# agent-charon/MinGraph-UNet

Measured on AMD Instinct MI355X. Metric: segmented Mpix/sec, full MinGraph-UNet forward (U-Net + patch-graph GAT), 512x512 batch, higher is better.
Workload: dtype f32

## Files before the change

### mingraph-unet_amd/csrc/convt_x3.hip

```cpp
#include <hip/hip_runtime.h>
#include <stdint.h>

#include <algorithm>
#include <type_traits>

#include "common.h"
#include "pack_small.h"

namespace mgu {

typedef float f32x16 __attribute__((ext_vector_type(16)));
typedef float f32x4 __attribute__((ext_vector_type(4)));
typedef unsigned u32x4 __attribute__((ext_vector_type(4)));
typedef __bf16 bf16x8 __attribute__((ext_vector_type(8)));

namespace {

__device__ __forceinline__ void split3_pack(const float a, const float b, unsigned& p0, unsigned& p1, unsigned& p2) {
  const unsigned ua = __float_as_uint(a), ub = __float_as_uint(b);
  p0 = __builtin_amdgcn_perm(ub, ua, 0x07060302u);
  const float ra = a - __uint_as_float(ua & 0xffff0000u), rb = b - __uint_as_float(ub & 0xffff0000u);
  const unsigned va = __float_as_uint(ra), vb = __float_as_uint(rb);
  p1 = __builtin_amdgcn_perm(vb, va, 0x07060302u);
  const float sa = ra - __uint_as_float(va & 0xffff0000u), sb = rb - __uint_as_float(vb & 0xffff0000u);
  p2 = __builtin_amdgcn_perm(__float_as_uint(sb), __float_as_uint(sa), 0x07060302u);
}

__device__ __forceinline__ f32x16 mfma_bf16(const u32x4 a, const u32x4 b, const f32x16 c) {
  return __builtin_amdgcn_mfma_f32_32x32x16_bf16(__builtin_bit_cast(bf16x8, a), __builtin_bit_cast(bf16x8, b), c, 0, 0, 0);
}

__global__ void pack_convt_x3_kernel(const float* __restrict__ w, uint16_t* __restrict__ Wx, int Cin, int Cout) {
  pack_convt_x3_body(w, Wx, Cin, Cout, 0, blockIdx.x, gridDim.x);
}

__device__ __forceinline__ void lds_barrier() { asm volatile("s_waitcnt lgkmcnt(0)\n\ts_barrier" ::: "memory"); }

template <int MODE, int NI>
__global__ __launch_bounds__(256, 2) void convt2x2_x3_kernel(const float* __restrict__ in, const int ldin, const uint16_t* __restrict__ Wx,
                                                             const float* __restrict__ shift, float* __restrict__ out, const int M,
                                                             const int H, const int W, const int Cin, const int Cout, const int ldout,
                                                             const int coff, const int Hout, const int Wout, const int ntn,
                                                             const int nblocks) {
  constexpr int AP = 40, ABUF = 3 * 128 * AP;
  __shared__ __attribute__((aligned(16))) uint16_t As[2 * ABUF];
  __shared__ int rowoff[128];
  const int chunk = gridDim.x >> 3;
  const int lb = (blockIdx.x & 7) * chunk + (blockIdx.x >> 3);
  if (lb >= nblocks) return;
  const int nt = lb % ntn, mt = lb / ntn;
  const int tid = threadIdx.x, lane = tid & 63, wave = tid >> 6;
  const int wm = wave >> 1, wn = wave & 1, lr = lane & 31, lh = lane >> 5;
  const int bm0 = mt * 128;
  const int HW = H * W;
  long long pix0;
  {
    const int img = bm0 / HW, rem = bm0 - img * HW, y = rem / W;
    pix0 = ((long long)img * Hout + 2 * y) * Wout + 2 * (rem - y * W);
  }
  if (tid < 128) {
    const int m = bm0 + tid;
    int off = 0;
    if (m < M) {
      const int img = m / HW, rem = m - img * HW, y = rem / W, x = rem - y * W;
      off = (int)((((long long)img * Hout + 2 * y) * Wout + 2 * x - pix0) * ldout);
    }
    rowoff[tid] = off;
  }

  const int arow = tid >> 3, ach = (tid & 7) * 4;
  const float* aptr[4];
#pragma unroll
  for (int j = 0; j < 4; ++j) {
    const int m = min(bm0 + j * 32 + arow, M - 1);
    if (MODE == 0) {
      aptr[j] = in + (size_t)m * ldin + ach;
    } else {
      const int img = m / HW, rem = m - img * HW, y = rem / W, x = rem - y * W;
      aptr[j] = in + (((size_t)img * Hout + 2 * y) * Wout + 2 * x) * ldin + ach;
    }
  }
  const int nk = (MODE == 0 ? Cin : 4 * Cin) >> 5;
  const int spq = Cin >> 5;
  auto koff = [&](int s) -> int {
    if (MODE == 0) return s * 32;
    const int q = s / spq;
    return ((q >> 1) * Wout + (q & 1)) * ldin + (s - q * spq) * 32;
  };
  f32x4 areg[2][4];
  auto load_a = [&](int s, auto set_t) {
    constexpr int set = decltype(set_t)::value;
    const int ko = koff(s);
#pragma unroll
    for (int j = 0; j < 4; ++j) areg[set][j] = *reinterpret_cast<const f32x4*>(aptr[j] + ko);
  };
  auto store_a = [&](int buf, auto set_t) {
    constexpr int set = decltype(set_t)::value;
    uint16_t* const base = As + buf * ABUF + arow * AP + ach;
#pragma unroll
    for (int j = 0; j < 4; ++j) {
      unsigned p[3][2];
      split3_pack(areg[set][j][0], areg[set][j][1], p[0][0], p[1][0], p[2][0]);
      split3_pack(areg[set][j][2], areg[set][j][3], p[0][1], p[1][1], p[2][1]);
#pragma unroll
      for (int q = 0; q < 3; ++q) *reinterpret_cast<uint2*>(base + (q * 128 + j * 32) * AP) = uint2{p[q][0], p[q][1]};
    }
  };

  const int nt128 = NI == 2 ? nt : nt >> 1, sub0 = NI == 2 ? wn * 2 : (nt & 1) * 2 + wn;
  const u32x4* const bp = reinterpret_cast<const u32x4*>(Wx) + ((size_t)nt128 * (2 * nk) * 12 + sub0 * 3) * 64 + lane;
  u32x4 br[2][3 * NI];
  auto load_b = [&](int kk, auto buf_t) {
    constexpr int buf = decltype(buf_t)::value;
#pragma unroll
    for (int f = 0; f < 3 * NI; ++f) br[buf][f] = bp[((size_t)kk * 12 + f) * 64];
  };

  f32x16 acc[2][NI];
#pragma unroll
  for (int mi = 0; mi < 2; ++mi)
#pragma unroll
    for (int ni = 0; ni < NI; ++ni)
#pragma unroll
      for (int r = 0; r < 16; ++r) acc[mi][ni][r] = 0.f;

  const int aoff = (wm * 64 + lr) * AP + lh * 8;
  auto half_step = [&](int buf, int ss, auto bb_t) {
    constexpr int bb = decltype(bb_t)::value;
    u32x4 pa[2][3];
#pragma unroll
    for (int mi = 0; mi < 2; ++mi)
#pragma unroll
      for (int q = 0; q < 3; ++q)
        pa[mi][q] = *reinterpret_cast<const u32x4*>(As + buf * ABUF + (q * 128 + mi * 32) * AP + aoff + ss * 16);
#pragma unroll
    for (int mi = 0; mi < 2; ++mi)
#pragma unroll
      for (int ni = 0; ni < NI; ++ni) {
        f32x16 t = acc[mi][ni];
        t = mfma_bf16(pa[mi][2], br[bb][ni * 3 + 0], t);
        t = mfma_bf16(pa[mi][0], br[bb][ni * 3 + 2], t);
        t = mfma_bf16(pa[mi][1], br[bb][ni * 3 + 1], t);
        t = mfma_bf16(pa[mi][1], br[bb][ni * 3 + 0], t);
        t = mfma_bf16(pa[mi][0], br[bb][ni * 3 + 1], t);
        t = mfma_bf16(pa[mi][0], br[bb][ni * 3 + 0], t);
        acc[mi][ni] = t;
      }
  };
  using B0 = std::integral_constant<int, 0>;
  using B1 = std::integral_constant<int, 1>;
  const int nkk = 2 * nk;
  load_a(0, B0{});
  load_a(min(1, nk - 1), B1{});
  load_b(0, B0{});
  store_a(0, B0{});
  lds_barrier();
  auto second_half_and_stage = [&](int buf, auto bb_t, auto set_t) {
    half_step(buf, 1, bb_t);
    store_a(buf ^ 1, set_t);
#pragma unroll
    for (int k = 0; k < 12 * NI; ++k) {
      __builtin_amdgcn_sched_group_barrier(0x008, 1, 0);
      __builtin_amdgcn_sched_group_barrier(0x002, NI == 2 ? 4 : 8, 0);
    }
    __builtin_amdgcn_sched_group_barrier(0x200, 12, 0);
  };
  for (int s = 0; s < nk; s += 2) {
    load_a(min(s + 2, nk - 1), B0{});
    load_b(min(2 * s + 1, nkk - 1), B1{});
    __builtin_amdgcn_sched_barrier(0);
    half_step(0, 0, B0{});
    load_b(min(2 * s + 2, nkk - 1), B0{});
    __builtin_amdgcn_sched_barrier(0);
    second_half_and_stage(0, B1{}, B1{});
    __builtin_amdgcn_sched_barrier(0);
    lds_barrier();
    if (s + 1 >= nk) break;
    load_a(min(s + 3, nk - 1), B1{});
    load_b(min(2 * s + 3, nkk - 1), B1{});
    __builtin_amdgcn_sched_barrier(0);
    half_step(1, 0, B0{});
    load_b(min(2 * s + 4, nkk - 1), B0{});
    __builtin_amdgcn_sched_barrier(0);
    second_half_and_stage(1, B1{}, B0{});
    __builtin_amdgcn_sched_barrier(0);
    lds_barrier();
  }

  float* const tile_out = MODE == 0 ? out + (size_t)pix0 * ldout + coff : out + (size_t)bm0 * ldout + coff;
  const bool full_m = bm0 + 128 <= M;
  auto store_tile = [&](auto guarded_t) {
    constexpr bool GUARDED = decltype(guarded_t)::value;
#pragma unroll
    for (int ni = 0; ni < NI; ++ni) {
      const int n = nt * (64 * NI) + wn * (32 * NI) + ni * 32 + lr;
      int ncol = n;
      if (MODE == 0) {
        const int q = n / Cout;
        ncol = ((q >> 1) * Wout + (q & 1)) * ldout + (n - q * Cout);
      }
      const float sh = shift ? shift[n] : 0.f;
#pragma unroll
      for (int mi = 0; mi < 2; ++mi)
#pragma unroll
        for (int r = 0; r < 16; ++r) {
          const int rrow = wm * 64 + mi * 32 + (r & 3) + 8 * (r >> 2) + 4 * lh;
          const unsigned idx = (unsigned)((MODE == 0 ? rowoff[rrow] : rrow * ldout) + ncol);
          const float v = acc[mi][ni][r] + sh;
          if (!GUARDED) tile_out[idx] = v;
          else if (bm0 + rrow < M) tile_out[idx] = v;
        }
    }
  };
  if (full_m) store_tile(std::false_type{});
  else store_tile(std::true_type{});
}

}

size_t convt_x3_floats(int Cin, int Cout) { return (size_t)Cin * Cout * 6; }


namespace {

__global__ void pack_convt_x3_dgrad_kernel(const float* __restrict__ w, uint16_t* __restrict__ Wx, int Cin, int Cout) {
  pack_convt_x3_body(w, Wx, Cin, Cout, 1, blockIdx.x, gridDim.x);
}

}

size_t convt_x3_dgrad_floats(int Cin, int Cout) { return (size_t)((Cin + 127) / 128 * 128) * Cout * 6; }

hipError_t launch_pack_convt_x3_dgrad(const float* w, float* Wx, int Cin, int Cout, hipStream_t s) {
  if ((Cin & 63) || (Cout & 31)) return hipErrorInvalidValue;
  hipLaunchKernelGGL(pack_convt_x3_dgrad_kernel, dim3((unsigned)std::min<int64_t>(4096, ((int64_t)Cin * Cout * 4 + 255) / 256)), dim3(256), 0, s, w,
                     reinterpret_cast<uint16_t*>(Wx), Cin, Cout);
  return hipGetLastError();
}

hipError_t launch_convt_x3_dgrad(const IgemmDesc& d, hipStream_t s) {
  const bool wide = (d.N & 127) == 0;
  const int mtiles = (d.M + 127) / 128, ntn = d.N / (wide ? 128 : 64);
  const int nb = mtiles * ntn;
  const int chunk = (nb + 7) / 8;
  if (wide)
    hipLaunchKernelGGL((convt2x2_x3_kernel<1, 2>), dim3(chunk * 8), dim3(256), 0, s, d.in, d.ldin, reinterpret_cast<const uint16_t*>(d.wu),
                       (const float*)nullptr, d.out, d.M, d.H, d.W, d.Cp, d.N, d.ldout, d.coff, d.Hout, d.Wout, ntn, nb);
  else
    hipLaunchKernelGGL((convt2x2_x3_kernel<1, 1>), dim3(chunk * 8), dim3(256), 0, s, d.in, d.ldin, reinterpret_cast<const uint16_t*>(d.wu),
                       (const float*)nullptr, d.out, d.M, d.H, d.W, d.Cp, d.N, d.ldout, d.coff, d.Hout, d.Wout, ntn, nb);
  return hipGetLastError();
}

hipError_t launch_pack_convt_x3(const float* w, float* Wx, int Cin, int Cout, hipStream_t s) {
  if ((Cin & 15) || (Cout & 31)) return hipErrorInvalidValue;
  hipLaunchKernelGGL(pack_convt_x3_kernel, dim3((unsigned)std::min<int64_t>(4096, ((int64_t)Cin * Cout * 4 + 255) / 256)), dim3(256), 0, s, w, reinterpret_cast<uint16_t*>(Wx), Cin,
                     Cout);
  return hipGetLastError();
}

hipError_t launch_convt_x3(const IgemmDesc& d, hipStream_t s) {
  const int mtiles = (d.M + 127) / 128, ntn = d.N / 128;
  const int nb = mtiles * ntn;
  const int chunk = (nb + 7) / 8;
  hipLaunchKernelGGL((convt2x2_x3_kernel<0, 2>), dim3(chunk * 8), dim3(256), 0, s, d.in, d.ldin, reinterpret_cast<const uint16_t*>(d.wu), d.shift, d.out,
                     d.M, d.H, d.W, d.Cp, d.ct_cout, d.ldout, d.coff, d.Hout, d.Wout, ntn, nb);
  return hipGetLastError();
}

}
```

Before: 798.0.

## Make transposed-conv x3 kernel persistent with cross-tile prefetch and LDS-staged stores

Specializes the MODE 0, NI 2 transposed-conv kernel into a persistent kernel. Grid size is capped at the resident workgroup count and each workgroup loops over its XCD chunk of tiles, prefetching the next tile's A and B operands while the current tile's epilogue runs. The epilogue transposes accumulators through LDS so that stores are 4-wide contiguous per row instead of scattered scalar writes. This targets launch-tail and epilogue overhead and store coalescing, at the cost of extra LDS traffic, more scheduling complexity and a host-side occupancy query cached per device.

```diff
diff --git a/mingraph-unet_amd/csrc/convt_x3.hip b/mingraph-unet_amd/csrc/convt_x3.hip
--- a/mingraph-unet_amd/csrc/convt_x3.hip
+++ b/mingraph-unet_amd/csrc/convt_x3.hip
@@ -2,6 +2,7 @@
 #include <stdint.h>
 
 #include <algorithm>
+#include <atomic>
 #include <type_traits>
 
 #include "common.h"
@@ -35,6 +36,12 @@
 }
 
 __device__ __forceinline__ void lds_barrier() { asm volatile("s_waitcnt lgkmcnt(0)\n\ts_barrier" ::: "memory"); }
+__device__ __forceinline__ void lds_barrier_fenced() {
+  asm volatile("" ::: "memory");
+  __builtin_amdgcn_s_waitcnt(0xC07F);
+  __builtin_amdgcn_s_barrier();
+  asm volatile("" ::: "memory");
+}
 
 template <int MODE, int NI>
 __global__ __launch_bounds__(256, 2) void convt2x2_x3_kernel(const float* __restrict__ in, const int ldin, const uint16_t* __restrict__ Wx,
@@ -216,6 +223,202 @@
   else store_tile(std::true_type{});
 }
 
+template <>
+__global__ __launch_bounds__(256, 2) void convt2x2_x3_kernel<0, 2>(const float* __restrict__ in, const int ldin, const uint16_t* __restrict__ Wx,
+                                                                   const float* __restrict__ shift, float* __restrict__ out, const int M,
+                                                                   const int H, const int W, const int Cin, const int Cout, const int ldout,
+                                                                   const int coff, const int Hout, const int Wout, const int ntn,
+                                                                   const int nblocks) {
+  constexpr int AP = 40, ABUF = 3 * 128 * AP;
+  __shared__ __attribute__((aligned(16))) uint16_t As[2 * ABUF];
+  __shared__ int rowoff[128];
+  const int per_xcd = gridDim.x >> 3, chunk = (nblocks + 7) >> 3;
+  const int xend = min(((int)blockIdx.x & 7) * chunk + chunk, nblocks);
+  int lb = (blockIdx.x & 7) * chunk + (blockIdx.x >> 3);
+  if (lb >= xend) return;
+  const int tid = threadIdx.x, lane = tid & 63, wave = __builtin_amdgcn_readfirstlane(tid >> 6);
+  const int wm = wave >> 1, wn = wave & 1, lr = lane & 31, lh = lane >> 5;
+  const int HW = H * W;
+  const int nk = Cin >> 5, nkk = 2 * nk;
+  const int arow = tid >> 3, ach = (tid & 7) * 4;
+
+  const float* aptr[4];
+  const u32x4* bp;
+  auto set_tile = [&](int t) {
+    const int bm = t / ntn * 128;
+#pragma unroll
+    for (int j = 0; j < 4; ++j) aptr[j] = in + (size_t)min(bm + j * 32 + arow, M - 1) * ldin + ach;
+    bp = reinterpret_cast<const u32x4*>(Wx) + ((size_t)(t % ntn) * nkk * 12 + wn * 6) * 64 + lane;
+  };
+  f32x4 areg[2][4];
+  auto load_a = [&](int s, auto set_t) {
+    constexpr int set = decltype(set_t)::value;
+#pragma unroll
+    for (int j = 0; j < 4; ++j) areg[set][j] = *reinterpret_cast<const f32x4*>(aptr[j] + s * 32);
+  };
+  auto store_a = [&](int buf, auto set_t) {
+    constexpr int set = decltype(set_t)::value;
+    uint16_t* const base = As + buf * ABUF + arow * AP + ach;
+#pragma unroll
+    for (int j = 0; j < 4; ++j) {
+      unsigned p[3][2];
+      split3_pack(areg[set][j][0], areg[set][j][1], p[0][0], p[1][0], p[2][0]);
+      split3_pack(areg[set][j][2], areg[set][j][3], p[0][1], p[1][1], p[2][1]);
+#pragma unroll
+      for (int q = 0; q < 3; ++q) *reinterpret_cast<uint2*>(base + (q * 128 + j * 32) * AP) = uint2{p[q][0], p[q][1]};
+    }
+  };
+  u32x4 br[2][6];
+  auto load_b = [&](int kk, auto buf_t) {
+    constexpr int buf = decltype(buf_t)::value;
+#pragma unroll
+    for (int f = 0; f < 6; ++f) br[buf][f] = bp[((size_t)kk * 12 + f) * 64];
+  };
+
+  f32x16 acc[2][2];
+  const int aoff = (wm * 64 + lr) * AP + lh * 8;
+  auto half_step = [&](int buf, int ss, auto bb_t) {
+    constexpr int bb = decltype(bb_t)::value;
+    u32x4 pa[2][3];
+#pragma unroll
+    for (int mi = 0; mi < 2; ++mi)
+#pragma unroll
+      for (int q = 0; q < 3; ++q)
+        pa[mi][q] = *reinterpret_cast<const u32x4*>(As + buf * ABUF + (q * 128 + mi * 32) * AP + aoff + ss * 16);
+#pragma unroll
+    for (int mi = 0; mi < 2; ++mi)
+#pragma unroll
+      for (int ni = 0; ni < 2; ++ni) {
+        f32x16 t = acc[mi][ni];
+        t = mfma_bf16(pa[mi][2], br[bb][ni * 3 + 0], t);
+        t = mfma_bf16(pa[mi][0], br[bb][ni * 3 + 2], t);
+        t = mfma_bf16(pa[mi][1], br[bb][ni * 3 + 1], t);
+        t = mfma_bf16(pa[mi][1], br[bb][ni * 3 + 0], t);
+        t = mfma_bf16(pa[mi][0], br[bb][ni * 3 + 1], t);
+        t = mfma_bf16(pa[mi][0], br[bb][ni * 3 + 0], t);
+        acc[mi][ni] = t;
+      }
+  };
+  using B0 = std::integral_constant<int, 0>;
+  using B1 = std::integral_constant<int, 1>;
+  auto second_half_and_stage = [&](int buf, auto bb_t, auto set_t) {
+    half_step(buf, 1, bb_t);
+    store_a(buf ^ 1, set_t);
+#pragma unroll
+    for (int k = 0; k < 24; ++k) {
+      __builtin_amdgcn_sched_group_barrier(0x008, 1, 0);
+      __builtin_amdgcn_sched_group_barrier(0x002, 4, 0);
+    }
+    __builtin_amdgcn_sched_group_barrier(0x200, 12, 0);
+  };
+  auto prologue_loads = [&]() {
+    load_a(0, B0{});
+    load_a(min(1, nk - 1), B1{});
+    load_b(0, B0{});
+  };
+
+  set_tile(lb);
+  prologue_loads();
+  store_a(0, B0{});
+  lds_barrier_fenced();
+  for (;;) {
+    const int nt = lb % ntn, bm0 = lb / ntn * 128;
+    long long pix0;
+    {
+      const int img = bm0 / HW, rem = bm0 - img * HW, y = rem / W;
+      pix0 = ((long long)img * Hout + 2 * y) * Wout + 2 * (rem - y * W);
+    }
+    if (tid < 128) {
+      const int m = bm0 + tid;
+      int off = 0;
+      if (m < M) {
+        const int img = m / HW, rem = m - img * HW, y = rem / W, x = rem - y * W;
+        off = (int)((((long long)img * Hout + 2 * y) * Wout + 2 * x - pix0) * ldout);
+      }
+      rowoff[tid] = off;
+    }
+#pragma unroll
+    for (int mi = 0; mi < 2; ++mi)
+#pragma unroll
+      for (int ni = 0; ni < 2; ++ni)
+#pragma unroll
+        for (int r = 0; r < 16; ++r) acc[mi][ni][r] = 0.f;
+
+    for (int s = 0; s < nk; s += 2) {
+      load_a(min(s + 2, nk - 1), B0{});
+      load_b(min(2 * s + 1, nkk - 1), B1{});
+      __builtin_amdgcn_sched_barrier(0);
+      half_step(0, 0, B0{});
+      load_b(min(2 * s + 2, nkk - 1), B0{});
+      __builtin_amdgcn_sched_barrier(0);
+      second_half_and_stage(0, B1{}, B1{});
+      __builtin_amdgcn_sched_barrier(0);
+      lds_barrier_fenced();
+      if (s + 1 < nk) {
+        load_a(min(s + 3, nk - 1), B1{});
+        load_b(min(2 * s + 3, nkk - 1), B1{});
+        __builtin_amdgcn_sched_barrier(0);
+        half_step(1, 0, B0{});
+        load_b(min(2 * s + 4, nkk - 1), B0{});
+        __builtin_amdgcn_sched_barrier(0);
+        second_half_and_stage(1, B1{}, B0{});
+        __builtin_amdgcn_sched_barrier(0);
+        lds_barrier_fenced();
+      }
+    }
+    const int lbn = lb + per_xcd;
+    const bool has_next = lbn < xend;
+    if (has_next) {
+      set_tile(lbn);
+      prologue_loads();
+    }
+
+    float* const tile_out = out + (size_t)pix0 * ldout + coff;
+    int ncol[2];
+    float sh[2];
+#pragma unroll
+    for (int ni = 0; ni < 2; ++ni) {
+      const int n0 = nt * 128 + wn * 64 + ni * 32, q = n0 / Cout;
+      ncol[ni] = ((q >> 1) * Wout + (q & 1)) * ldout + (n0 - q * Cout);
+      sh[ni] = shift ? shift[n0 + lr] : 0.f;
+    }
+    {
+      int el = lane;
+      asm volatile("" : "+v"(el));
+      const int elr = el & 31, elh = el >> 5, trow = el >> 3, tcol = (el & 7) * 4;
+      float* const Ts = reinterpret_cast<float*>(As + ABUF) + wave * 1024;
+#pragma unroll
+      for (int mi = 0; mi < 2; ++mi) {
+        int ro[4];
+#pragma unroll
+        for (int it = 0; it < 4; ++it) ro[it] = rowoff[wm * 64 + mi * 32 + it * 8 + trow];
+#pragma unroll
+        for (int ni = 0; ni < 2; ++ni) {
+#pragma unroll
+          for (int r = 0; r < 16; ++r) Ts[((r & 3) + 8 * (r >> 2) + 4 * elh) * 32 + elr] = acc[mi][ni][r] + sh[ni];
+          asm volatile("s_waitcnt lgkmcnt(0)" ::: "memory");
+          __builtin_amdgcn_wave_barrier();
+#pragma unroll
+          for (int it = 0; it < 4; ++it) {
+            const f32x4 v = *reinterpret_cast<const f32x4*>(Ts + (it * 8 + trow) * 32 + tcol);
+            if (bm0 + wm * 64 + mi * 32 + it * 8 + trow < M) {
+              float* const p = tile_out + ro[it] + ncol[ni] + tcol;
+#pragma unroll
+              for (int c = 0; c < 4; ++c) p[c] = v[c];
+            }
+          }
+          asm volatile("s_waitcnt lgkmcnt(0)" ::: "memory");
+          __builtin_amdgcn_wave_barrier();
+        }
+      }
+    }
+    if (!has_next) break;
+    store_a(0, B0{});
+    lds_barrier_fenced();
+    lb = lbn;
+  }
+}
+
 }
 
 size_t convt_x3_floats(int Cin, int Cout) { return (size_t)Cin * Cout * 6; }
@@ -262,8 +465,21 @@
 hipError_t launch_convt_x3(const IgemmDesc& d, hipStream_t s) {
   const int mtiles = (d.M + 127) / 128, ntn = d.N / 128;
   const int nb = mtiles * ntn;
-  const int chunk = (nb + 7) / 8;
-  hipLaunchKernelGGL((convt2x2_x3_kernel<0, 2>), dim3(chunk * 8), dim3(256), 0, s, d.in, d.ldin, reinterpret_cast<const uint16_t*>(d.wu), d.shift, d.out,
+  static std::atomic<int> resident_of[64];
+  int dev = 0;
+  (void)hipGetDevice(&dev);
+  std::atomic<int>& slot = resident_of[dev >= 0 && dev < 64 ? dev : 0];
+  int resident = slot.load(std::memory_order_relaxed);
+  if (!resident) {
+    int cus = 256, occ = 2;
+    (void)hipDeviceGetAttribute(&cus, hipDeviceAttributeMultiprocessorCount, dev);
+    if (hipOccupancyMaxActiveBlocksPerMultiprocessor(&occ, reinterpret_cast<const void*>(&convt2x2_x3_kernel<0, 2>), 256, 0) != hipSuccess || occ < 1)
+      occ = 2;
+    resident = std::max(8, cus * occ / 8 * 8);
+    slot.store(resident, std::memory_order_relaxed);
+  }
+  const int nwg = std::min((nb + 7) / 8 * 8, resident);
+  hipLaunchKernelGGL((convt2x2_x3_kernel<0, 2>), dim3(nwg), dim3(256), 0, s, d.in, d.ldin, reinterpret_cast<const uint16_t*>(d.wu), d.shift, d.out,
                      d.M, d.H, d.W, d.Cp, d.ct_cout, d.ldout, d.coff, d.Hout, d.Wout, ntn, nb);
   return hipGetLastError();
 }
```

Result: no change. 799.1, median of 6 (+0.1%).
